# pashtari/factorizer

Measured on AMD Instinct MI355X. Metric: volumes/sec fwd+bwd, Swin Factorizer 128^3, higher is better.
Workload: dtype f32

## Files before the change

### factorizer_amd/_native.py

```python
from __future__ import annotations

import ctypes
import os
import threading

import torch

_HERE = os.path.dirname(os.path.abspath(__file__))
LIB_PATH = os.environ.get("FZ_LIB_PATH") or os.path.join(_HERE, "libfactorizer_hip.so")

FZ_OK = 0
FZ_E_UNSUPPORTED = -2
ABI_VERSION = 7
SOLVER_ID = {"mu": 0, "hals": 1, "cd": 2, "smu": 3}
STORE_F32, STORE_BF16 = 0, 1
PRODUCTS_DEFAULT, PRODUCTS_SPLIT_BF16, PRODUCTS_FP32_MFMA = 0, 1, 2
_products = threading.local()


def products() -> int:
    return getattr(_products, "value", PRODUCTS_DEFAULT)


class use_products:
# ... 171 lines not shown
    "fz_gcorr_supported": ([_i] * 5, _i),
    "fz_gcorr": ([_vp] * 5 + [_i] * 11 + [_f, _vp], _i),
    "fz_gcorr_wgrad_workspace_bytes": ([_i] * 10, _i64),
    "fz_gcorr_wgrad": ([_vp] * 4 + [_i] * 11 + [_vp], _i),
    "fz_gnmf_supported": ([_i, _i64, _i, _i, _i], _i),
    "fz_gnmf_workspace_bytes": ([_i64, _i, _i64, _i, _i, _i], _i64),
    "fz_gnmf_launches": ([_i, _i, _i], _i),
    "fz_gnmf_fwd": ([_vp] * 6 + [_i64, _i, _i64, _i, _i, _i, _f, _vp, _vp], _i),
    "fz_gnmf_bwd": ([_vp] * 7 + [_i64, _i, _i64, _i, _i, _i, _i, _f, _vp, _vp], _i),
    "fz_nmf_cf_supported": ([_i] * 11, _i),
    "fz_nmf_cf_fwd": ([_vp] * 4 + [_i] * 5 + [_c.POINTER(_i)] + [_i] * 5 + [_f, _i, _vp], _i),
    "fz_nmf_cf_bwd": ([_vp] * 5 + [_i] * 5 + [_c.POINTER(_i)] + [_i] * 7 + [_f, _i, _vp], _i),
    "fz_nmf_cf_factors_supported": ([_i] * 12 + [_c.POINTER(_i)], _i),
    "fz_nmf_cf_fwd_store_factors": ([_vp] * 5 + [_i] * 5 + [_c.POINTER(_i)] + [_i] * 3 + [_f, _i, _vp], _i),
    "fz_nmf_cf_fwd_from_factors": ([_vp] * 6 + [_i] * 5 + [_c.POINTER(_i)] * 2 + [_i] * 4 + [_f, _i, _vp], _i),
    "fz_nmf_pcf_supported": ([_i] * 11, _i),
    "fz_nmf_pcf_fwd": ([_vp] * 4 + [_i] * 8 + [_c.POINTER(_i)] + [_i] * 5 + [_f, _i, _vp], _i),
    "fz_nmf_pcf_bwd": ([_vp] * 5 + [_i] * 8 + [_c.POINTER(_i)] + [_i] * 7 + [_f, _i, _vp], _i),
    "fz_nmf_pcf_bwd_prefers_separate": ([_i] * 4, _i),
    "fz_act_add": ([_vp, _vp, _i64, _i, _vp], _i),
    "fz_mlp_pre_supported": ([_i, _i, _i64, _i], _i),
    "fz_mlp_drop_supported": ([_i, _i, _i64, _i], _i),
    "fz_mlp_chain_drop": ([_c.POINTER(MlpDesc), _c.POINTER(MlpDropout), _vp], _i),
    "fz_conv3_prologue_supported": ([_i] * 4, _i),
    "fz_conv3_fwd2": ([_vp] * 4 + [_i] * 8 + [_c.POINTER(BlockPrologue), _vp], _i),
    "fz_upcat2": ([_vp, _vp, _vp, _i, _vp, _vp, _vp] + [_i] * 7 + [_c.POINTER(BlockPrologue), _vp], _i),
    "fz_gemm": ([_c.POINTER(GemmDesc), _vp], _i),
    "fz_gemm_bx_enable": ([_i], _i),
    "fz_gemm_lnbwd_partials": ([_c.POINTER(GemmDesc)], _i64),
    "fz_reduce_rows": ([_vp, _i64, _i, _vp, _vp, _vp], _i),
# ... 65 lines not shown
```

### factorizer_amd/csrc/nmf_cf.h

```cpp
#pragma once
#include <cstdlib>

#include "fz_common.h"
#include "nmf_core.h"
#include "nmf_gram.h"

namespace fz {

struct CfGeom {
  int B, C, D, H, W;
  int h;
  int G0, G1, G2;
  int s0, s1, s2;
  int accumulate;
  int divisor;
  float gscale_div;
  int64_t plane;
  int ps0, ps1, ps2;
};

enum { CF_PLAIN = 0, CF_STORE_FACTORS = 1, CF_FROM_FACTORS = 2 };

struct CfWave {
  using F = float;
  int lane;
  __device__ __forceinline__ int col(int j) const {
    const int jp = j >> 2, e = j & 3;
    return (((jp * 4 + (lane >> 4)) * 8 + ((lane >> 1) & 7)) * 8) + (lane & 1) * 4 + e;
  }
  __device__ __forceinline__ float sum(float v) const { return wave_sum(v); }
  __device__ __forceinline__ void sum8(float (&v)[8]) const { wave_sum8(v, lane); }
  __device__ __forceinline__ void st_priv(float* base, int idx, float v) const { base[idx * 64 + lane] = v; }
  __device__ __forceinline__ float ld_priv(const float* base, int idx) const { return base[idx * 64 + lane]; }
  __device__ __forceinline__ void st_uni(float* base, int idx, float v) const {
    if (lane == 0) base[idx] = v;
  }
// ... 260 lines not shown
#pragma unroll
    for (int c = 0; c < 2; ++c) {
      const float4 a0 = *reinterpret_cast<const float4*>(S + c * 64 * TL::LW + own0);
      const float4 a1 = *reinterpret_cast<const float4*>(S + c * 64 * TL::LW + own1);
      x[2 * s + c][0] = a0.x; x[2 * s + c][1] = a0.y; x[2 * s + c][2] = a0.z; x[2 * s + c][3] = a0.w;
      x[2 * s + c][4] = a1.x; x[2 * s + c][5] = a1.y; x[2 * s + c][6] = a1.z; x[2 * s + c][7] = a1.w;
    }
    __syncthreads();
  }
}


template <typename AT>
int cf_bwd_gram_launch(const AT* t, const float* v0, const AT* ga, AT* gt, const CfGeom& q, int64_t nmat, int T, int G,
                       float eps, int xcd_remap, hipStream_t st);

}
```

### factorizer_amd/csrc/nmf_cf.hip

```cpp
#include "nmf_cf.h"

namespace fz {

template <int R, int SOLVER, int WPB, bool HALF, typename AT, int FORM>
__device__ __forceinline__ void cf_fwd_tile_body(const AT* __restrict__ t, const float* __restrict__ u0,
                                                 const float* __restrict__ v0, AT* __restrict__ out, float* vfac, float* ufac,
                                                 const CfGeom& q, const CfTileId& id, int T, float eps, float* S) {
  static_assert(FORM == CF_PLAIN || (R == 1 && WPB == 8 && !HALF), "the factor forms: rank 1, 8 patches per workgroup, W-axis shifts = 0 (mod 4)");
  using TL = CfTile<WPB>;
  const int tid = threadIdx.x, lane = tid & 63, wave = tid >> 6;
  int64_t base, V;
  unsigned off[2], off2[2];
  int lidx[2];
  cf_tile_decode<WPB>(q, id, tid, base, V, off, lidx, off2);
  const int own0 = cf_owner_lidx<WPB>(lane, wave, 0), own1 = cf_owner_lidx<WPB>(lane, wave, 1);

  float x[8][8];
#pragma unroll
  for (int dd = 0; dd < 8; ++dd)
#pragma unroll
    for (int k = 0; k < 2; ++k) {
      const float4 v = cf_ld4<HALF>(t + base + dd * V, off[k], off2[k]);
      x[dd][k * 4 + 0] = v.x; x[dd][k * 4 + 1] = v.y; x[dd][k * 4 + 2] = v.z; x[dd][k * 4 + 3] = v.w;
    }
// ... 397 lines not shown
  const int64_t nmat = (int64_t)B * q.h * q.G0 * q.G1 * q.G2;
  if (nmat >= (int64_t)1 << 31) return fail(FZ_E_UNSUPPORTED, "fz_nmf_cf: more than 2^31 matrices");
  const int per_wave = (R == 1 ? Hist<8, 8, 1>::floats(G) : Hist<8, 8, 2>::floats(G)) * (int)sizeof(float);
  if (per_wave > 160 * 1024) return fail(FZ_E_UNSUPPORTED, "fz_nmf_cf_bwd: history exceeds LDS");
  int wpb = 65536 / per_wave;
  if (wpb > 4) wpb = 4;
  if (wpb > 8) wpb = 8;
  if (wpb < 1) wpb = 1;
  const int xr = 1 | (tile_order() << 1);
  hipStream_t st = (hipStream_t)stream;
  const int tile = FZ_KNOB("FZ_CF_TILE_BWD").set ? FZ_KNOB("FZ_CF_TILE_BWD").val : 1;
  const bool half = (q.s2 % 4) != 0;
  if (half || (tile && (q.G2 % 4) == 0)) {
    const int twpb = (q.G2 % 4) == 0 ? 4 : 1;
    const bool gram_on = !(FZ_KNOB("FZ_CF_GRAM").set && FZ_KNOB("FZ_CF_GRAM").val == 0);
    const bool gram_wins = !(sizeof(AT) == 4 && accumulate && nmat >= 32768);
    if (gram_on && gram_wins && R == 1 && solver == FZ_SOLVER_HALS && relu_gate && G >= 1) {
      rc = cf_bwd_gram_launch<AT>(t, v0, ga, gt, q, nmat, T, G, eps, xr, st);
      if (rc != FZ_E_UNSUPPORTED) return rc;
    }
    const int tlds = (twpb == 4 ? CfTile<4>::STAGE_FLOATS : CfTile<1>::STAGE_FLOATS) * (int)sizeof(float) + per_wave * twpb;
    if (tlds > 160 * 1024) {
      if (half) return fail(FZ_E_UNSUPPORTED, "fz_nmf_cf_bwd: history exceeds LDS for a W-axis shift of 2 (mod 4)");
    } else {
      const unsigned nblk = (unsigned)(nmat / twpb);
#define FZ_CF_BWD_TILE(RR, SS, WW, HH)                                                                      \
  do {                                                                                                      \
    auto kern = nmf_cf_bwd_tile_kernel<RR, SS, WW, HH, AT>;                                                    \
    if (tlds > 65536)                                                                                       \
      FZ_HIP_OK(hipFuncSetAttribute(reinterpret_cast<const void*>(kern),                                    \
                                    hipFuncAttributeMaxDynamicSharedMemorySize, tlds));                     \
// ... 14 lines not shown
  dim3 grid((unsigned)((nmat + wpb - 1) / wpb)), block(64 * wpb);
#define FZ_CF_BWD(RR, SS)                                                                                 \
  do {                                                                                                    \
    auto kern = nmf_cf_bwd_kernel<RR, SS, AT>;                                                          \
    if (lds > 65536)                                                                                      \
      FZ_HIP_OK(hipFuncSetAttribute(reinterpret_cast<const void*>(kern),                                  \
                                    hipFuncAttributeMaxDynamicSharedMemorySize, lds));                    \
    hipLaunchKernelGGL(kern, grid, block, lds, st, t, u0, v0, ga, gt, q, nmat, T, G, eps, relu_gate, xr);     \
  } while (0)
  if (R == 1) { FZ_SOLVER_CASES(FZ_CF_BWD, 1); }
  else { FZ_SOLVER_CASES(FZ_CF_BWD, 2); }
  FZ_LAUNCH_CHECK();
  return FZ_OK;
}

extern "C" int fz_nmf_cf_bwd(const void* t, const float* u0, const float* v0, const void* ga, void* gt, int B,
                             int C, int D, int H, int W, const int* shift, int accumulate, int nshift,
                             int relu_gate, int R, int T, int Tgrad, int solver, float eps, int act_dtype,
                             fz_stream_t stream) {
  if (act_dtype == FZ_STORE_F32)
    return cf_bwd_launch<float>((const float*)t, u0, v0, (const float*)ga, (float*)gt, B, C, D, H, W, shift, accumulate,
                                nshift, relu_gate, R, T, Tgrad, solver, eps, stream);
  if (act_dtype == FZ_STORE_BF16)
    return cf_bwd_launch<bf16>((const bf16*)t, u0, v0, (const bf16*)ga, (bf16*)gt, B, C, D, H, W, shift, accumulate,
                               nshift, relu_gate, R, T, Tgrad, solver, eps, stream);
  return fail(FZ_E_ARG, "fz_nmf_cf_bwd: bad act_dtype");
}
```

### factorizer_amd/csrc/nmf_cf_gram.hip

```cpp
#include "nmf_cf.h"
#include "nmf_gram.h"

#ifndef FZ_GRAM_WAVES
#define FZ_GRAM_WAVES 3
#endif

namespace fz {

enum { CFG_HALVES = 0, CFG_RAW = 2 };

#ifdef FZ_PROBE_GRAM_NOMATH
#define FZ_GRAM_OUT_ROW(m, grow) probe_acc += grow[(m) & 7]
#else
#define FZ_GRAM_OUT_ROW(m, grow) P.out_row(m, grow)
#endif

template <typename AT> struct CfRaw;
template <> struct CfRaw<float> { using T = float4; };
template <> struct CfRaw<bf16> { using T = uint2; };

template <bool HALF>
__device__ __forceinline__ float4 cf_ld_raw(const float* p, unsigned o, unsigned o2) { return cf_ld4<HALF>(p, o, o2); }
template <bool HALF>
__device__ __forceinline__ uint2 cf_ld_raw(const bf16* p, unsigned o, unsigned o2) {
  if (HALF) {
    const unsigned a = *reinterpret_cast<const unsigned*>(cf_at(p, o)), b = *reinterpret_cast<const unsigned*>(cf_at(p, o2));
    return make_uint2(a, b);
  }
  return *reinterpret_cast<const uint2*>(cf_at(p, o));
}
__device__ __forceinline__ float4 cf_raw_f4(const float4& v) { return v; }
__device__ __forceinline__ float4 cf_raw_f4(const uint2& v) {
  return make_float4(__uint_as_float(v.x << 16), __uint_as_float(v.x & 0xffff0000u), __uint_as_float(v.y << 16),
                     __uint_as_float(v.y & 0xffff0000u));
}

template <int WPB, bool HALF, typename AT, int MODE>
__global__ __launch_bounds__(WPB * 64, WPB == 4 ? FZ_GRAM_WAVES : 1) void nmf_cf_bwd_gram_kernel(
    const AT* __restrict__ t, const float* __restrict__ v0, const AT* __restrict__ ga, AT* __restrict__ gt, CfGeom q,
    int T, int G, float eps, int xcd_remap) {
  extern __shared__ __attribute__((aligned(16))) float fz_lds_cfg[];
  using TL = CfTile<WPB>;
  using Raw = typename CfRaw<AT>::T;
  constexpr int NB = MODE == CFG_RAW ? 8 : 4;
  constexpr int IMG = 64 * TL::LW;
  float* S = fz_lds_cfg;
  const CfTileId id = cf_tile_id<WPB>(q, cf_logical_block(xcd_remap));
  const int tid = threadIdx.x, lane = tid & 63, wave = tid >> 6;
  int64_t base, V;
  unsigned off[2], off2[2];
  int lidx[2];
  cf_tile_decode<WPB>(q, id, tid, base, V, off, lidx, off2);
  const int own0 = cf_owner_lidx<WPB>(lane, wave, 0), own1 = cf_owner_lidx<WPB>(lane, wave, 1);
  float* hist = S + TL::STAGE_FLOATS + wave * gram_hist_floats(G - 1);

  float x[8][8];
#pragma unroll
  for (int dd = 0; dd < 8; ++dd)
#pragma unroll
    for (int k = 0; k < 2; ++k) {
      const float4 v = cf_ld4<HALF>(t + base + dd * V, off[k], off2[k]);
      x[dd][k * 4 + 0] = v.x; x[dd][k * 4 + 1] = v.y; x[dd][k * 4 + 2] = v.z; x[dd][k * 4 + 3] = v.w;
    }
  cf_to_owner<WPB>(S, lidx, own0, own1, x);

  CfWave w{lane};
  GramBwd<8, CfWave> P;
  Raw gq[NB][2];
  auto request_g = [&]() {
#pragma unroll
    for (int dd = 0; dd < NB; ++dd)
#pragma unroll
      for (int k = 0; k < 2; ++k) gq[dd][k] = cf_ld_raw<HALF>(ga + base + dd * V, off[k], off2[k]);
  };
#ifdef FZ_PROBE_GRAM_NOMATH
  float probe_acc = 0.f;
  request_g();
#else
  P.forward(w, x, v0, 8, 512, T, G, eps, hist, request_g);
#endif
  asm volatile("" : "+s"(base));
#pragma unroll
  for (int bt = 0; bt < 8 / NB; ++bt) {
#pragma unroll
    for (int s = 0; s < NB / 2; ++s) {
#pragma unroll
      for (int c = 0; c < 2; ++c)
#pragma unroll
        for (int k = 0; k < 2; ++k) *reinterpret_cast<float4*>(S + c * IMG + lidx[k]) = cf_raw_f4(gq[2 * s + c][k]);
      if (MODE == CFG_HALVES && bt == 0 && s == NB / 2 - 1) {
#pragma unroll
        for (int dd = 0; dd < NB; ++dd)
#pragma unroll
          for (int k = 0; k < 2; ++k) gq[dd][k] = cf_ld_raw<HALF>(ga + base + (NB + dd) * V, off[k], off2[k]);
      }
      __syncthreads();
#pragma unroll
      for (int c = 0; c < 2; ++c) {
        const float4 a0 = *reinterpret_cast<const float4*>(S + c * IMG + own0);
        const float4 a1 = *reinterpret_cast<const float4*>(S + c * IMG + own1);
        const float grow[8] = {a0.x, a0.y, a0.z, a0.w, a1.x, a1.y, a1.z, a1.w};
        FZ_GRAM_OUT_ROW(NB * bt + 2 * s + c, grow);
      }
      __syncthreads();
    }
  }
#ifdef FZ_PROBE_GRAM_NOMATH
#else
  P.reverse(w, x, 1.0f / q.gscale_div, [] {});
#endif
#pragma unroll
  for (int bt = 0; bt < 8 / NB; ++bt) {
#pragma unroll
    for (int s = 0; s < NB / 2; ++s) {
      Raw old[2][2];
      if (q.accumulate) {
#pragma unroll
        for (int c = 0; c < 2; ++c)
#pragma unroll
          for (int k = 0; k < 2; ++k) old[c][k] = cf_ld_raw<HALF>(gt + base + (NB * bt + 2 * s + c) * V, off[k], off2[k]);
      }
#pragma unroll
      for (int c = 0; c < 2; ++c) {
        const int m = NB * bt + 2 * s + c;
        float o[8];
#ifdef FZ_PROBE_GRAM_NOMATH
#pragma unroll
        for (int e = 0; e < 8; ++e) o[e] = x[m][e] + probe_acc;
#else
        float srow[8], gsm, ga1m;
        P.row_coeffs(w, m, srow, gsm, ga1m);
        P.gx_row(m, x, srow, gsm, ga1m, o);
#endif
#pragma unroll
        for (int e = 0; e < 8; ++e) o[e] = x[m][e] > 0.f ? o[e] : 0.f;
        *reinterpret_cast<float4*>(S + c * IMG + own0) = make_float4(o[0], o[1], o[2], o[3]);
        *reinterpret_cast<float4*>(S + c * IMG + own1) = make_float4(o[4], o[5], o[6], o[7]);
      }
      __syncthreads();
#pragma unroll
      for (int c = 0; c < 2; ++c)
#pragma unroll
        for (int k = 0; k < 2; ++k) {
          float4 z = *reinterpret_cast<const float4*>(S + c * IMG + lidx[k]);
          if (q.accumulate) {
            const float4 o = cf_raw_f4(old[c][k]);
            z.x += o.x; z.y += o.y; z.z += o.z; z.w += o.w;
          }
          cf_st4<HALF>(gt + base + (NB * bt + 2 * s + c) * V, off[k], off2[k], z);
        }
      __syncthreads();
    }
  }
}

template <typename AT>
int cf_bwd_gram_launch(const AT* t, const float* v0, const AT* ga, AT* gt, const CfGeom& q, int64_t nmat, int T, int G,
                       float eps, int xcd_remap, hipStream_t st) {
  const bool half = (q.s2 % 4) != 0;
#ifdef FZ_PROBE_GRAM_WPB
  const int twpb = (q.G2 % FZ_PROBE_GRAM_WPB) == 0 ? FZ_PROBE_GRAM_WPB : ((q.G2 % 4) == 0 ? 4 : 1);
#else
  const int twpb = (q.G2 % 4) == 0 ? 4 : 1;
#endif
  constexpr bool kF32 = sizeof(AT) == 4;
#ifdef FZ_PROBE_GRAM_WPB
  const int stage = twpb == FZ_PROBE_GRAM_WPB ? CfTile<FZ_PROBE_GRAM_WPB>::STAGE_FLOATS : (twpb == 4 ? CfTile<4>::STAGE_FLOATS : CfTile<1>::STAGE_FLOATS);
#else
// ... 10 lines not shown
#ifdef FZ_PROBE_GRAM_WPB
  if (!half && twpb == FZ_PROBE_GRAM_WPB) {
    auto kern = nmf_cf_bwd_gram_kernel<FZ_PROBE_GRAM_WPB, false, AT, kRegMode>;
    if (glds > 64 * 1024) FZ_HIP_OK(hipFuncSetAttribute(reinterpret_cast<const void*>(kern), hipFuncAttributeMaxDynamicSharedMemorySize, glds));
    FZ_CF_BWD_GRAM(FZ_PROBE_GRAM_WPB, false, kRegMode);
    FZ_LAUNCH_CHECK();
    return FZ_OK;
  }
#endif
  if (half) { if (twpb == 4) FZ_CF_BWD_GRAM(4, true, kRegMode); else FZ_CF_BWD_GRAM(1, true, kRegMode); }
  else if (twpb == 4) FZ_CF_BWD_GRAM(4, false, kRegMode);
  else return FZ_E_UNSUPPORTED;
  FZ_LAUNCH_CHECK();
  return FZ_OK;
}
template int cf_bwd_gram_launch<float>(const float*, const float*, const float*, float*, const CfGeom&, int64_t, int, int, float, int, hipStream_t);
template int cf_bwd_gram_launch<bf16>(const bf16*, const float*, const bf16*, bf16*, const CfGeom&, int64_t, int, int, float, int, hipStream_t);

}
```

### factorizer_amd/csrc/nmf_gram.h

```cpp
#pragma once

#include "nmf_core.h"

namespace fz {

FZ_HD int gram_hist_floats(int steps) { return 64 + (steps > 0 ? steps : 0) * 12; }

template <int NPL, class W>
struct GramBwd {
  using F = typename W::F;
  F vs[NPL];
  F gc[NPL];
  F vT[NPL];
  F gv[NPL];
  F col[8];
  F Kd[8];
  F gKd[8];
  F sd;
  F ud;
  F gsd, ga1d;
  F uT[8];
  F r;
  F binv;
  float eps, neps2;
// ... 186 lines not shown
#pragma unroll
      for (int k = 0; k < 8; ++k) gKd[k] = gKd[k] + gp * uk[k] + uo * gpk[k];
      un = uo;
    }
    ga1d = gud * binv;
  }

  FZ_HD void row_coeffs(W& w, int m, F (&srow)[8], F& gsm, F& ga1m) const {
#pragma unroll
    for (int k = 0; k < 8; ++k) srow[k] = w.grp_take(gKd[k], m);
    gsm = w.grp_take(gsd, m);
    ga1m = w.grp_take(ga1d, m);
  }
  FZ_HD void gx_row(int m, const F (&x)[8][NPL], const F (&srow)[8], const F& gsm, const F& ga1m, F (&out)[NPL]) const {
#pragma unroll
    for (int j = 0; j < NPL; ++j) {
      F acc = uT[m] * gc[j] + gsm;
      acc = acc + ga1m * vs[j];
#pragma unroll
      for (int k = 0; k < 8; ++k) acc = acc + srow[k] * x[k][j];
      out[j] = acc;
    }
  }
};

}
```

### factorizer_amd/functional.py

```python
from __future__ import annotations

import math
import os

import torch

from . import _native as N


def _dev_guard(t: torch.Tensor):
    return torch.cuda.device(t.device)


class KernelTimer:

    def __init__(self, only=None):
        self.records = []
        self.only = None if only is None else set(only)

    def launch(self, name, nbytes, fn, cols=0, flops=0):
        if self.only is not None and name not in self.only:
            return fn()
        s = torch.cuda.Event(enable_timing=True)
        e = torch.cuda.Event(enable_timing=True)
# ... 320 lines not shown

def nmf_cf_supported(geo: Geometry, R, T, G) -> bool:
    if len(geo.spatial) != 3 or any(s[2] % 2 for s in geo.shifts):
        return False
    return bool(N.lib().fz_nmf_cf_supported(geo.C, *geo.spatial, geo.d, *geo.patch, int(R), int(T), int(G)))


def nmf_cf_factors_supported(geo: Geometry, R, T, G) -> bool:
    if len(geo.spatial) != 3:
        return False
    k = (int(R), int(T), int(G))
    ok = geo._factors_ok.get(k)
    if ok is None:
        ok = geo._factors_ok[k] = bool(N.lib().fz_nmf_cf_factors_supported(geo.C, *geo.spatial, geo.d, *geo.patch, *k,
                                                                          geo.nshift, geo._carr))
    return ok


def nmf_pcf_supported(geo: Geometry, R, T, G) -> bool:
    if os.environ.get("FZ_NMF_PCF", "1") == "0":
        return False
    return bool(N.lib().fz_nmf_pcf_supported(geo.C, *geo.s3, geo.d, *geo.p3, int(R), int(T), int(G)))


def nmf_core_supported(geo: Geometry, R, T, G) -> bool:
    return nmf_cf_supported(geo, R, T, G) or nmf_pcf_supported(geo, R, T, G)


class FactCoreFn(torch.autograd.Function):

# ... 50 lines not shown
        t, u0, v0 = ctx.saved_tensors
        geo, T, G, solver, eps, relu_gate = ctx.cfg
        if G <= 0:
            return (torch.zeros_like(t),) + (None,) * 8
        ga = ga.contiguous()
        if ga.dtype != t.dtype:
            ga = ga.to(t.dtype)
        gt = torch.empty_like(t)
        B = t.shape[0]
        R = u0.shape[1]
        es = t.element_size()
        nb = 3 * es * t.numel()
        ad = N.act_dtype(t)
        hot = nmf_cf_supported(geo, R, T, G)
        with _dev_guard(t):
            for w, s in enumerate(geo.shifts3):
                arr = (N._i * 3)(*s)
                N.set_tile_order(w & 1)
                if hot:
                    rc = _timed(f"nmf_cf_bwd_{geo.C}x" + "x".join(str(v) for v in geo.spatial), nb + (es * t.numel() if w else 0), cols=t.numel() // geo.C, fn=lambda: N.lib().fz_nmf_cf_bwd(
                        t.data_ptr(), u0.data_ptr(), v0.data_ptr(), ga.data_ptr(), gt.data_ptr(), B, geo.C,
                        *geo.spatial, arr, int(w > 0), geo.nshift, int(relu_gate), R, T, G, N.SOLVER_ID[solver], eps,
                        ad, N.stream_ptr(t)))
                elif w > 0 and N.lib().fz_nmf_pcf_bwd_prefers_separate(*geo.p3, ad):
                    tmp = torch.empty_like(gt)
                    rc = _timed(f"nmf_pcf_bwd_{geo.C}x" + "x".join(str(v) for v in geo.spatial), nb, cols=t.numel() // geo.C, fn=lambda: N.lib().fz_nmf_pcf_bwd(
                        t.data_ptr(), u0.data_ptr(), v0.data_ptr(), ga.data_ptr(), tmp.data_ptr(), B, geo.C,
                        *geo.s3, *geo.p3, arr, 0, geo.nshift, int(relu_gate), R, T, G, N.SOLVER_ID[solver], eps,
                        ad, N.stream_ptr(t)))
                    N.check(rc, "fz_nmf_pcf_bwd")
# ... 251 lines not shown
```

### include/factorizer_hip.h

```cpp
#ifndef FACTORIZER_HIP_H
#define FACTORIZER_HIP_H

#include <stdint.h>

#ifdef __cplusplus
extern "C" {
#endif

#define FZ_OK 0
#define FZ_E_SHAPE (-1)
#define FZ_E_UNSUPPORTED (-2)
#define FZ_E_HIP (-3)
#define FZ_E_ARG (-4)

#define FZ_STORE_F32 0
#define FZ_STORE_BF16 1

#define FZ_SOLVER_MU 0
#define FZ_SOLVER_HALS 1
#define FZ_SOLVER_CD 2
#define FZ_SOLVER_SMU 3

typedef void* fz_stream_t;

// ... 41 lines not shown
                  int H, int W, const int* shift, int accumulate, int divisor, int R, int T,
                  int solver, float eps, int act_dtype, fz_stream_t stream);
int fz_nmf_cf_bwd(const void* t, const float* u0, const float* v0, const void* ga, void* gt, int B,
                  int C, int D, int H, int W, const int* shift, int accumulate, int nshift,
                  int relu_gate, int R, int T, int Tgrad, int solver, float eps, int act_dtype,
                  fz_stream_t stream);

int fz_nmf_cf_factors_supported(int C, int D, int H, int W, int d, int pd, int ph, int pw, int R, int T, int Tgrad,
                                int nshift, const int* shifts);
int fz_nmf_cf_fwd_store_factors(const void* t, const float* u0, const float* v0, float* vfac, float* ufac, int B,
                                int C, int D, int H, int W, const int* shift, int R, int T, int solver, float eps,
                                int act_dtype, fz_stream_t stream);
int fz_nmf_cf_fwd_from_factors(const void* t, const float* u0, const float* v0, const float* vfac, const float* ufac,
                               void* out, int B, int C, int D, int H, int W, const int* shift, const int* prev_shift,
                               int divisor, int R, int T, int solver, float eps, int act_dtype, fz_stream_t stream);

int fz_nmf_pcf_supported(int C, int D, int H, int W, int d, int pd, int ph, int pw, int R, int T, int Tgrad);
int fz_nmf_pcf_fwd(const void* t, const float* u0, const float* v0, void* out, int B, int C, int D, int H, int W,
                   int pd, int ph, int pw, const int* shift, int accumulate, int divisor, int R, int T, int solver,
                   float eps, int act_dtype, fz_stream_t stream);
int fz_nmf_pcf_bwd(const void* t, const float* u0, const float* v0, const void* ga, void* gt, int B, int C, int D,
                   int H, int W, int pd, int ph, int pw, const int* shift, int accumulate, int nshift, int relu_gate,
                   int R, int T, int Tgrad, int solver, float eps, int act_dtype, fz_stream_t stream);
int fz_nmf_pcf_bwd_prefers_separate(int pd, int ph, int pw, int act_dtype);
int fz_act_add(void* dst, const void* src, int64_t n, int act_dtype, fz_stream_t stream);

#define FZ_LOAD_PLAIN 0
#define FZ_LOAD_S2D 1
#define FZ_LOAD_K3 2
#define FZ_EPI_PLAIN 0
// ... 292 lines not shown
```

Before: 130.3.

## Fuse two-window NMF backward via stored per-patch factors instead of accumulate passes

Adds a factor-form backward for the shifted-window NMF. The first window's gram backward stores compact per-patch coefficients (gc image plus an 88-float cofactor record). The second window's kernel reconstructs the first window's input gradient from those factors and adds it in registers. This removes the separate accumulate read-modify-write of gt and one full pass over it, at the cost of extra factor storage, LDS staging and more arithmetic in the second kernel. The gram kernel body is moved into a shared include so both forms reuse it.

Measured after the change: 132.9 (median of 6 runs). 2.1% higher.

```diff
diff --git a/factorizer_amd/_native.py b/factorizer_amd/_native.py
--- a/factorizer_amd/_native.py
+++ b/factorizer_amd/_native.py
@@ -209,6 +209,9 @@
     "fz_nmf_cf_factors_supported": ([_i] * 12 + [_c.POINTER(_i)], _i),
     "fz_nmf_cf_fwd_store_factors": ([_vp] * 5 + [_i] * 5 + [_c.POINTER(_i)] + [_i] * 3 + [_f, _i, _vp], _i),
     "fz_nmf_cf_fwd_from_factors": ([_vp] * 6 + [_i] * 5 + [_c.POINTER(_i)] * 2 + [_i] * 4 + [_f, _i, _vp], _i),
+    "fz_nmf_cf_bwd_factors_supported": ([_i] * 14 + [_c.POINTER(_i)], _i),
+    "fz_nmf_cf_bwd_store_factors": ([_vp] * 5 + [_i] * 5 + [_c.POINTER(_i)] + [_i] * 3 + [_f, _i, _vp], _i),
+    "fz_nmf_cf_bwd_from_factors": ([_vp] * 6 + [_i] * 5 + [_c.POINTER(_i)] * 2 + [_i] * 3 + [_f, _i, _vp], _i),
     "fz_nmf_pcf_supported": ([_i] * 11, _i),
     "fz_nmf_pcf_fwd": ([_vp] * 4 + [_i] * 8 + [_c.POINTER(_i)] + [_i] * 5 + [_f, _i, _vp], _i),
     "fz_nmf_pcf_bwd": ([_vp] * 5 + [_i] * 8 + [_c.POINTER(_i)] + [_i] * 7 + [_f, _i, _vp], _i),
diff --git a/factorizer_amd/csrc/nmf_cf.h b/factorizer_amd/csrc/nmf_cf.h
--- a/factorizer_amd/csrc/nmf_cf.h
+++ b/factorizer_amd/csrc/nmf_cf.h
@@ -20,6 +20,7 @@
 };
 
 enum { CF_PLAIN = 0, CF_STORE_FACTORS = 1, CF_FROM_FACTORS = 2 };
+constexpr int CFG_COFAC = 88;
 
 struct CfWave {
   using F = float;
@@ -310,5 +311,8 @@
 template <typename AT>
 int cf_bwd_gram_launch(const AT* t, const float* v0, const AT* ga, AT* gt, const CfGeom& q, int64_t nmat, int T, int G,
                        float eps, int xcd_remap, hipStream_t st);
-
-}
+template <typename AT>
+int cf_bwd_gram_factors_launch(const AT* t, const float* v0, const AT* ga, AT* gt, float* gcfac, float* cofac, const CfGeom& q,
+                               int64_t nmat, int form, int T, int G, float eps, int xcd_remap, hipStream_t st);
+
+}
diff --git a/factorizer_amd/csrc/nmf_cf.hip b/factorizer_amd/csrc/nmf_cf.hip
--- a/factorizer_amd/csrc/nmf_cf.hip
+++ b/factorizer_amd/csrc/nmf_cf.hip
@@ -435,7 +435,7 @@
   if (half || (tile && (q.G2 % 4) == 0)) {
     const int twpb = (q.G2 % 4) == 0 ? 4 : 1;
     const bool gram_on = !(FZ_KNOB("FZ_CF_GRAM").set && FZ_KNOB("FZ_CF_GRAM").val == 0);
-    const bool gram_wins = !(sizeof(AT) == 4 && accumulate && nmat >= 32768);
+    const bool gram_wins = !(sizeof(AT) == 4 && accumulate && nmat >= 32768) || (FZ_KNOB("FZ_CF_GRAM").set && FZ_KNOB("FZ_CF_GRAM").val == 2);
     if (gram_on && gram_wins && R == 1 && solver == FZ_SOLVER_HALS && relu_gate && G >= 1) {
       rc = cf_bwd_gram_launch<AT>(t, v0, ga, gt, q, nmat, T, G, eps, xr, st);
       if (rc != FZ_E_UNSUPPORTED) return rc;
@@ -480,6 +480,74 @@
   return FZ_OK;
 }
 
+extern "C" int fz_nmf_cf_bwd_factors_supported(int C, int D, int H, int W, int d, int pd, int ph, int pw, int R, int T, int Tgrad,
+                                               int solver, int relu_gate, int nshift, const int* shifts) {
+  if (FZ_KNOB("FZ_CF_BWD_FACTORS").set && FZ_KNOB("FZ_CF_BWD_FACTORS").val == 0) return 0;
+  if (!fz_nmf_cf_factors_supported(C, D, H, W, d, pd, ph, pw, R, T, Tgrad, nshift, shifts)) return 0;
+  if (solver != FZ_SOLVER_HALS || !relu_gate) return 0;
+  if (T < 1 || Tgrad < T) return 0;
+  if ((C / 8) * (int64_t)(D / 8) * (H / 8) * (W / 8) >= ((int64_t)1 << 31)) return 0;
+  const int lds = (CfTile<4>::STAGE_FLOATS + 4 * gram_hist_floats(T - 1) + 4 * 8 * CFG_COFAC) * (int)sizeof(float);
+  return lds <= 64 * 1024 ? 1 : 0;
+}
+
+template <typename AT>
+static int cf_bwd_factors_launch(const AT* t, const float* v0, const AT* ga, AT* gt, float* gcfac, float* cofac, int B, int C,
+                                 int D, int H, int W, const int* shift, const int* prev_shift, int form, int nshift, int T,
+                                 int Tgrad, float eps, fz_stream_t stream, const char* who) {
+  CfGeom q;
+  int rc = cf_geom(q, B, C, D, H, W, shift, form == CF_FROM_FACTORS, 1);
+  if (rc != FZ_OK) return rc;
+  if (!t || !v0 || !ga || !gcfac || !cofac || (form == CF_FROM_FACTORS && (!gt || !prev_shift))) return fail(FZ_E_ARG, who);
+  if (W % 64) return fail(FZ_E_UNSUPPORTED, "fz_nmf_cf_bwd factor forms: W must be a multiple of 64");
+  if (nshift != 2) return fail(FZ_E_UNSUPPORTED, "fz_nmf_cf_bwd factor forms: exactly two windows");
+  if (T < 1 || Tgrad < T) return fail(FZ_E_UNSUPPORTED, "fz_nmf_cf_bwd factor forms: every iteration graded (1 <= T <= Tgrad)");
+  if (q.s2 % 4) return fail(FZ_E_UNSUPPORTED, "fz_nmf_cf_bwd factor forms: W-axis shift must be a multiple of 4");
+  if (form == CF_FROM_FACTORS) {
+    int ps[3];
+    cf_norm_shift(prev_shift, D, H, W, ps);
+    if (ps[2] % 4) return fail(FZ_E_UNSUPPORTED, "fz_nmf_cf_bwd factor forms: W-axis shift must be a multiple of 4");
+    q.ps0 = ps[0]; q.ps1 = ps[1]; q.ps2 = ps[2];
+  }
+  if (B == 0) return FZ_OK;
+  q.gscale_div = (float)nshift;
+  const int64_t nmat = (int64_t)B * q.h * q.G0 * q.G1 * q.G2;
+  if (nmat >= (int64_t)1 << 31) return fail(FZ_E_UNSUPPORTED, "fz_nmf_cf: more than 2^31 matrices");
+  const int xr = 1 | (tile_order() << 1);
+  rc = cf_bwd_gram_factors_launch<AT>(t, v0, ga, gt, gcfac, cofac, q, nmat, form, T, T, eps, xr, (hipStream_t)stream);
+  if (rc == FZ_E_UNSUPPORTED) return fail(rc, "fz_nmf_cf_bwd factor forms: history exceeds the LDS budget");
+  return rc;
+}
+
+extern "C" int fz_nmf_cf_bwd_store_factors(const void* t, const float* v0, const void* ga, float* gcfac, float* cofac, int B,
+                                           int C, int D, int H, int W, const int* shift, int nshift, int T, int Tgrad,
+                                           float eps, int act_dtype, fz_stream_t stream) {
+  const char* who = "fz_nmf_cf_bwd_store_factors: null pointer (t, v0, ga, gcfac or cofac)";
+  if (act_dtype == FZ_STORE_F32)
+    return cf_bwd_factors_launch<float>((const float*)t, v0, (const float*)ga, nullptr, gcfac, cofac, B, C, D, H, W, shift,
+                                        nullptr, CF_STORE_FACTORS, nshift, T, Tgrad, eps, stream, who);
+  if (act_dtype == FZ_STORE_BF16)
+    return cf_bwd_factors_launch<bf16>((const bf16*)t, v0, (const bf16*)ga, nullptr, gcfac, cofac, B, C, D, H, W, shift,
+                                       nullptr, CF_STORE_FACTORS, nshift, T, Tgrad, eps, stream, who);
+  return fail(FZ_E_ARG, "fz_nmf_cf_bwd_store_factors: bad act_dtype");
+}
+
+extern "C" int fz_nmf_cf_bwd_from_factors(const void* t, const float* v0, const void* ga, const float* gcfac,
+                                          const float* cofac, void* gt, int B, int C, int D, int H, int W, const int* shift,
+                                          const int* prev_shift, int nshift, int T, int Tgrad, float eps, int act_dtype,
+                                          fz_stream_t stream) {
+  const char* who = "fz_nmf_cf_bwd_from_factors: null pointer (t, v0, ga, gcfac, cofac, gt or prev_shift)";
+  if (act_dtype == FZ_STORE_F32)
+    return cf_bwd_factors_launch<float>((const float*)t, v0, (const float*)ga, (float*)gt, const_cast<float*>(gcfac),
+                                        const_cast<float*>(cofac), B, C, D, H, W, shift, prev_shift, CF_FROM_FACTORS, nshift, T,
+                                        Tgrad, eps, stream, who);
+  if (act_dtype == FZ_STORE_BF16)
+    return cf_bwd_factors_launch<bf16>((const bf16*)t, v0, (const bf16*)ga, (bf16*)gt, const_cast<float*>(gcfac),
+                                       const_cast<float*>(cofac), B, C, D, H, W, shift, prev_shift, CF_FROM_FACTORS, nshift, T,
+                                       Tgrad, eps, stream, who);
+  return fail(FZ_E_ARG, "fz_nmf_cf_bwd_from_factors: bad act_dtype");
+}
+
 extern "C" int fz_nmf_cf_bwd(const void* t, const float* u0, const float* v0, const void* ga, void* gt, int B,
                              int C, int D, int H, int W, const int* shift, int accumulate, int nshift,
                              int relu_gate, int R, int T, int Tgrad, int solver, float eps, int act_dtype,
diff --git a/factorizer_amd/csrc/nmf_cf_gram.hip b/factorizer_amd/csrc/nmf_cf_gram.hip
--- a/factorizer_amd/csrc/nmf_cf_gram.hip
+++ b/factorizer_amd/csrc/nmf_cf_gram.hip
@@ -35,123 +35,35 @@
                      __uint_as_float(v.y & 0xffff0000u));
 }
 
+template <typename AT>
+__device__ __forceinline__ float cf_as_stored(float v) {
+  if constexpr (sizeof(AT) == 2) {
+    const f32v4 f = {v, v, v, v};
+    const f32v4 r = __builtin_convertvector(__builtin_convertvector(f, bf16v4), f32v4);
+    return r[0];
+  }
+  return v;
+}
+
 template <int WPB, bool HALF, typename AT, int MODE>
 __global__ __launch_bounds__(WPB * 64, WPB == 4 ? FZ_GRAM_WAVES : 1) void nmf_cf_bwd_gram_kernel(
     const AT* __restrict__ t, const float* __restrict__ v0, const AT* __restrict__ ga, AT* __restrict__ gt, CfGeom q,
     int T, int G, float eps, int xcd_remap) {
   extern __shared__ __attribute__((aligned(16))) float fz_lds_cfg[];
-  using TL = CfTile<WPB>;
-  using Raw = typename CfRaw<AT>::T;
-  constexpr int NB = MODE == CFG_RAW ? 8 : 4;
-  constexpr int IMG = 64 * TL::LW;
-  float* S = fz_lds_cfg;
-  const CfTileId id = cf_tile_id<WPB>(q, cf_logical_block(xcd_remap));
-  const int tid = threadIdx.x, lane = tid & 63, wave = tid >> 6;
-  int64_t base, V;
-  unsigned off[2], off2[2];
-  int lidx[2];
-  cf_tile_decode<WPB>(q, id, tid, base, V, off, lidx, off2);
-  const int own0 = cf_owner_lidx<WPB>(lane, wave, 0), own1 = cf_owner_lidx<WPB>(lane, wave, 1);
-  float* hist = S + TL::STAGE_FLOATS + wave * gram_hist_floats(G - 1);
+  constexpr int FORM = CF_PLAIN;
+  float* const gcfac = nullptr;
+  float* const cofac = nullptr;
+#include "nmf_cf_gram_body.inc"
+}
 
-  float x[8][8];
-#pragma unroll
-  for (int dd = 0; dd < 8; ++dd)
-#pragma unroll
-    for (int k = 0; k < 2; ++k) {
-      const float4 v = cf_ld4<HALF>(t + base + dd * V, off[k], off2[k]);
-      x[dd][k * 4 + 0] = v.x; x[dd][k * 4 + 1] = v.y; x[dd][k * 4 + 2] = v.z; x[dd][k * 4 + 3] = v.w;
-    }
-  cf_to_owner<WPB>(S, lidx, own0, own1, x);
-
-  CfWave w{lane};
-  GramBwd<8, CfWave> P;
-  Raw gq[NB][2];
-  auto request_g = [&]() {
-#pragma unroll
-    for (int dd = 0; dd < NB; ++dd)
-#pragma unroll
-      for (int k = 0; k < 2; ++k) gq[dd][k] = cf_ld_raw<HALF>(ga + base + dd * V, off[k], off2[k]);
-  };
-#ifdef FZ_PROBE_GRAM_NOMATH
-  float probe_acc = 0.f;
-  request_g();
-#else
-  P.forward(w, x, v0, 8, 512, T, G, eps, hist, request_g);
-#endif
-  asm volatile("" : "+s"(base));
-#pragma unroll
-  for (int bt = 0; bt < 8 / NB; ++bt) {
-#pragma unroll
-    for (int s = 0; s < NB / 2; ++s) {
-#pragma unroll
-      for (int c = 0; c < 2; ++c)
-#pragma unroll
-        for (int k = 0; k < 2; ++k) *reinterpret_cast<float4*>(S + c * IMG + lidx[k]) = cf_raw_f4(gq[2 * s + c][k]);
-      if (MODE == CFG_HALVES && bt == 0 && s == NB / 2 - 1) {
-#pragma unroll
-        for (int dd = 0; dd < NB; ++dd)
-#pragma unroll
-          for (int k = 0; k < 2; ++k) gq[dd][k] = cf_ld_raw<HALF>(ga + base + (NB + dd) * V, off[k], off2[k]);
-      }
-      __syncthreads();
-#pragma unroll
-      for (int c = 0; c < 2; ++c) {
-        const float4 a0 = *reinterpret_cast<const float4*>(S + c * IMG + own0);
-        const float4 a1 = *reinterpret_cast<const float4*>(S + c * IMG + own1);
-        const float grow[8] = {a0.x, a0.y, a0.z, a0.w, a1.x, a1.y, a1.z, a1.w};
-        FZ_GRAM_OUT_ROW(NB * bt + 2 * s + c, grow);
-      }
-      __syncthreads();
-    }
-  }
-#ifdef FZ_PROBE_GRAM_NOMATH
-#else
-  P.reverse(w, x, 1.0f / q.gscale_div, [] {});
-#endif
-#pragma unroll
-  for (int bt = 0; bt < 8 / NB; ++bt) {
-#pragma unroll
-    for (int s = 0; s < NB / 2; ++s) {
-      Raw old[2][2];
-      if (q.accumulate) {
-#pragma unroll
-        for (int c = 0; c < 2; ++c)
-#pragma unroll
-          for (int k = 0; k < 2; ++k) old[c][k] = cf_ld_raw<HALF>(gt + base + (NB * bt + 2 * s + c) * V, off[k], off2[k]);
-      }
-#pragma unroll
-      for (int c = 0; c < 2; ++c) {
-        const int m = NB * bt + 2 * s + c;
-        float o[8];
-#ifdef FZ_PROBE_GRAM_NOMATH
-#pragma unroll
-        for (int e = 0; e < 8; ++e) o[e] = x[m][e] + probe_acc;
-#else
-        float srow[8], gsm, ga1m;
-        P.row_coeffs(w, m, srow, gsm, ga1m);
-        P.gx_row(m, x, srow, gsm, ga1m, o);
-#endif
-#pragma unroll
-        for (int e = 0; e < 8; ++e) o[e] = x[m][e] > 0.f ? o[e] : 0.f;
-        *reinterpret_cast<float4*>(S + c * IMG + own0) = make_float4(o[0], o[1], o[2], o[3]);
-        *reinterpret_cast<float4*>(S + c * IMG + own1) = make_float4(o[4], o[5], o[6], o[7]);
-      }
-      __syncthreads();
-#pragma unroll
-      for (int c = 0; c < 2; ++c)
-#pragma unroll
-        for (int k = 0; k < 2; ++k) {
-          float4 z = *reinterpret_cast<const float4*>(S + c * IMG + lidx[k]);
-          if (q.accumulate) {
-            const float4 o = cf_raw_f4(old[c][k]);
-            z.x += o.x; z.y += o.y; z.z += o.z; z.w += o.w;
-          }
-          cf_st4<HALF>(gt + base + (NB * bt + 2 * s + c) * V, off[k], off2[k], z);
-        }
-      __syncthreads();
-    }
-  }
+template <typename AT, int MODE, int FORM>
+__global__ __launch_bounds__(256, FZ_GRAM_WAVES) void nmf_cf_bwd_gram_fac_kernel(
+    const AT* __restrict__ t, const float* __restrict__ v0, const AT* __restrict__ ga, AT* __restrict__ gt,
+    float* __restrict__ gcfac, float* __restrict__ cofac, CfGeom q, int T, int G, float eps, int xcd_remap) {
+  extern __shared__ __attribute__((aligned(16))) float fz_lds_cfg[];
+  constexpr int WPB = 4;
+  constexpr bool HALF = false;
+#include "nmf_cf_gram_body.inc"
 }
 
 template <typename AT>
@@ -192,6 +104,27 @@
   FZ_LAUNCH_CHECK();
   return FZ_OK;
 }
+template <typename AT>
+int cf_bwd_gram_factors_launch(const AT* t, const float* v0, const AT* ga, AT* gt, float* gcfac, float* cofac, const CfGeom& q,
+                               int64_t nmat, int form, int T, int G, float eps, int xcd_remap, hipStream_t st) {
+  if ((q.s2 % 4) || (q.ps2 % 4) || (q.G2 % 4) || G != T || G < 1) return FZ_E_UNSUPPORTED;
+  int glds = (CfTile<4>::STAGE_FLOATS + 4 * gram_hist_floats(G - 1)) * (int)sizeof(float);
+  if (form == CF_FROM_FACTORS) glds += 4 * 8 * CFG_COFAC * (int)sizeof(float);
+  if (glds > 64 * 1024) return FZ_E_UNSUPPORTED;
+  const unsigned nblk = (unsigned)(nmat / 4);
+  constexpr int kRegMode = sizeof(AT) == 4 ? CFG_HALVES : CFG_RAW;
+  if (form == CF_STORE_FACTORS)
+    hipLaunchKernelGGL((nmf_cf_bwd_gram_fac_kernel<AT, kRegMode, CF_STORE_FACTORS>), dim3(nblk), dim3(256), glds, st, t, v0, ga,
+                       gt, gcfac, cofac, q, T, G, eps, xcd_remap);
+  else
+    hipLaunchKernelGGL((nmf_cf_bwd_gram_fac_kernel<AT, kRegMode, CF_FROM_FACTORS>), dim3(nblk), dim3(256), glds, st, t, v0, ga,
+                       gt, gcfac, cofac, q, T, G, eps, xcd_remap);
+  FZ_LAUNCH_CHECK();
+  return FZ_OK;
+}
+template int cf_bwd_gram_factors_launch<float>(const float*, const float*, const float*, float*, float*, float*, const CfGeom&, int64_t, int, int, int, float, int, hipStream_t);
+template int cf_bwd_gram_factors_launch<bf16>(const bf16*, const float*, const bf16*, bf16*, float*, float*, const CfGeom&, int64_t, int, int, int, float, int, hipStream_t);
+
 template int cf_bwd_gram_launch<float>(const float*, const float*, const float*, float*, const CfGeom&, int64_t, int, int, float, int, hipStream_t);
 template int cf_bwd_gram_launch<bf16>(const bf16*, const float*, const bf16*, bf16*, const CfGeom&, int64_t, int, int, float, int, hipStream_t);
 
diff --git a/factorizer_amd/csrc/nmf_cf_gram_body.inc b/factorizer_amd/csrc/nmf_cf_gram_body.inc
--- /dev/null
+++ b/factorizer_amd/csrc/nmf_cf_gram_body.inc
@@ -0,0 +1,207 @@
+  static_assert(FORM == CF_PLAIN || (WPB == 4 && !HALF), "the factor forms: 4 patches per workgroup, W-axis shifts = 0 (mod 4)");
+  using TL = CfTile<WPB>;
+  using Raw = typename CfRaw<AT>::T;
+  constexpr int NB = MODE == CFG_RAW ? 8 : 4;
+  constexpr int IMG = 64 * TL::LW;
+  float* S = fz_lds_cfg;
+  const CfTileId id = cf_tile_id<WPB>(q, cf_logical_block(xcd_remap));
+  const int tid = threadIdx.x, lane = tid & 63, wave = tid >> 6;
+  int64_t base, V;
+  unsigned off[2], off2[2];
+  int lidx[2];
+  cf_tile_decode<WPB>(q, id, tid, base, V, off, lidx, off2);
+  const int own0 = cf_owner_lidx<WPB>(lane, wave, 0), own1 = cf_owner_lidx<WPB>(lane, wave, 1);
+  float* hist = S + TL::STAGE_FLOATS + wave * gram_hist_floats(G - 1);
+
+  float x[8][8];
+#pragma unroll
+  for (int dd = 0; dd < 8; ++dd)
+#pragma unroll
+    for (int k = 0; k < 2; ++k) {
+      const float4 v = cf_ld4<HALF>(t + base + dd * V, off[k], off2[k]);
+      x[dd][k * 4 + 0] = v.x; x[dd][k * 4 + 1] = v.y; x[dd][k * 4 + 2] = v.z; x[dd][k * 4 + 3] = v.w;
+    }
+  const int64_t bh = (int64_t)id.b * q.h + id.hh;
+  const int64_t vol = (int64_t)q.D * q.H * q.W;
+  const float* co[2];
+  unsigned vcol[2];
+  if constexpr (FORM == CF_FROM_FACTORS) {
+    float* stage = S + TL::STAGE_FLOATS + WPB * gram_hist_floats(G - 1) + wave * (8 * CFG_COFAC);
+    const int gp[3] = {id.g0, id.g1, id.gq * WPB + wave}, sh[3] = {q.s0, q.s1, q.s2}, ps[3] = {q.ps0, q.ps1, q.ps2};
+    const int dim[3] = {q.D, q.H, q.W}, ng[3] = {q.G0, q.G1, q.G2};
+    int o[3], pa[3][2];
+#pragma unroll
+    for (int a = 0; a < 3; ++a) {
+      o[a] = gp[a] * 8 - sh[a] + ps[a];
+      if (o[a] < 0) o[a] += dim[a];
+      if (o[a] >= dim[a]) o[a] -= dim[a];
+      pa[a][0] = o[a] >> 3;
+      pa[a][1] = pa[a][0] + 1 == ng[a] ? 0 : pa[a][0] + 1;
+    }
+    const float* cp = cofac + bh * q.G0 * q.G1 * q.G2 * CFG_COFAC;
+#pragma unroll
+    for (int r = 0; r < 3; ++r) {
+      const int i = lane + 64 * r, lp = i / (CFG_COFAC / 4), c4 = i % (CFG_COFAC / 4);
+      if (i < 8 * (CFG_COFAC / 4)) {
+        const int pidx = (pa[0][(lp >> 2) & 1] * q.G1 + pa[1][(lp >> 1) & 1]) * q.G2 + pa[2][lp & 1];
+        *reinterpret_cast<float4*>(stage + lp * CFG_COFAC + c4 * 4) = ld4(cp + (int64_t)pidx * CFG_COFAC + c4 * 4);
+      }
+    }
+    __builtin_amdgcn_fence(__ATOMIC_ACQ_REL, "wavefront");
+    const int p12 = (lane >> 1) & 7, p2 = (lane & 1) * 4;
+    int c1 = o[1] + p12; if (c1 >= q.H) c1 -= q.H;
+    int c2 = o[2] + p2; if (c2 >= q.W) c2 -= q.W;
+    const int b1 = (c1 >> 3) != pa[1][0], b2 = (c2 >> 3) != pa[2][0];
+#pragma unroll
+    for (int jp = 0; jp < 2; ++jp) {
+      int c0 = o[0] + jp * 4 + (lane >> 4); if (c0 >= q.D) c0 -= q.D;
+      const int b0 = (c0 >> 3) != pa[0][0];
+      co[jp] = stage + (b0 * 4 + b1 * 2 + b2) * CFG_COFAC;
+      vcol[jp] = (unsigned)((((c0 & 7) * 8 + (c1 & 7)) * 8) + (c2 & 7));
+    }
+  }
+  cf_to_owner<WPB>(S, lidx, own0, own1, x);
+
+  CfWave w{lane};
+  GramBwd<8, CfWave> P;
+  Raw gq[NB][2];
+  auto request_g = [&]() {
+#pragma unroll
+    for (int dd = 0; dd < NB; ++dd)
+#pragma unroll
+      for (int k = 0; k < 2; ++k) gq[dd][k] = cf_ld_raw<HALF>(ga + base + dd * V, off[k], off2[k]);
+  };
+#ifdef FZ_PROBE_GRAM_NOMATH
+  float probe_acc = 0.f;
+  request_g();
+#else
+  P.forward(w, x, v0, 8, 512, T, G, eps, hist, request_g);
+#endif
+  asm volatile("" : "+s"(base));
+#pragma unroll
+  for (int bt = 0; bt < 8 / NB; ++bt) {
+#pragma unroll
+    for (int s = 0; s < NB / 2; ++s) {
+#pragma unroll
+      for (int c = 0; c < 2; ++c)
+#pragma unroll
+        for (int k = 0; k < 2; ++k) *reinterpret_cast<float4*>(S + c * IMG + lidx[k]) = cf_raw_f4(gq[2 * s + c][k]);
+      if (MODE == CFG_HALVES && bt == 0 && s == NB / 2 - 1) {
+#pragma unroll
+        for (int dd = 0; dd < NB; ++dd)
+#pragma unroll
+          for (int k = 0; k < 2; ++k) gq[dd][k] = cf_ld_raw<HALF>(ga + base + (NB + dd) * V, off[k], off2[k]);
+      }
+      __syncthreads();
+#pragma unroll
+      for (int c = 0; c < 2; ++c) {
+        const float4 a0 = *reinterpret_cast<const float4*>(S + c * IMG + own0);
+        const float4 a1 = *reinterpret_cast<const float4*>(S + c * IMG + own1);
+        const float grow[8] = {a0.x, a0.y, a0.z, a0.w, a1.x, a1.y, a1.z, a1.w};
+        FZ_GRAM_OUT_ROW(NB * bt + 2 * s + c, grow);
+      }
+      __syncthreads();
+    }
+  }
+  float4 gcq[2];
+  auto request_gc0 = [&] {
+    if constexpr (FORM == CF_FROM_FACTORS) {
+#pragma unroll
+      for (int k = 0; k < 2; ++k) gcq[k] = ld4(cf_at(gcfac + bh * vol, off[k]));
+    }
+  };
+#ifdef FZ_PROBE_GRAM_NOMATH
+  request_gc0();
+#else
+  P.reverse(w, x, 1.0f / q.gscale_div, request_gc0);
+#endif
+  if constexpr (FORM == CF_STORE_FACTORS) {
+    *reinterpret_cast<float4*>(S + own0) = make_float4(P.gc[0], P.gc[1], P.gc[2], P.gc[3]);
+    *reinterpret_cast<float4*>(S + own1) = make_float4(P.gc[4], P.gc[5], P.gc[6], P.gc[7]);
+    __syncthreads();
+    float* gp = gcfac + bh * vol;
+#pragma unroll
+    for (int k = 0; k < 2; ++k) st4(cf_at(gp, off[k]), *reinterpret_cast<const float4*>(S + lidx[k]));
+    if ((lane & 7) == 0) {
+      const int g = lane >> 3;
+      float* cp = cofac + ((((bh * q.G0 + id.g0) * q.G1 + id.g1) * q.G2 + id.gq * WPB + wave) * CFG_COFAC);
+      cp[g] = P.ud;
+      cp[8 + g] = P.gsd;
+      cp[16 + g] = P.ga1d;
+      st4(cp + 24 + g * 8, make_float4(P.gKd[0], P.gKd[1], P.gKd[2], P.gKd[3]));
+      st4(cp + 24 + g * 8 + 4, make_float4(P.gKd[4], P.gKd[5], P.gKd[6], P.gKd[7]));
+    }
+    return;
+  }
+  float gc0[8], vs0[8];
+  if constexpr (FORM == CF_FROM_FACTORS) {
+#pragma unroll
+    for (int k = 0; k < 2; ++k) *reinterpret_cast<float4*>(S + lidx[k]) = gcq[k];
+#pragma unroll
+    for (int jp = 0; jp < 2; ++jp) {
+#pragma unroll
+      for (int e = 0; e < 4; ++e) vs0[jp * 4 + e] = v0[vcol[jp] + e];
+    }
+    __syncthreads();
+    const float4 a0 = *reinterpret_cast<const float4*>(S + own0), a1 = *reinterpret_cast<const float4*>(S + own1);
+    gc0[0] = a0.x; gc0[1] = a0.y; gc0[2] = a0.z; gc0[3] = a0.w; gc0[4] = a1.x; gc0[5] = a1.y; gc0[6] = a1.z; gc0[7] = a1.w;
+    __syncthreads();
+  }
+#pragma unroll
+  for (int bt = 0; bt < 8 / NB; ++bt) {
+#pragma unroll
+    for (int s = 0; s < NB / 2; ++s) {
+      Raw old[2][2];
+      if (FORM == CF_PLAIN && q.accumulate) {
+#pragma unroll
+        for (int c = 0; c < 2; ++c)
+#pragma unroll
+          for (int k = 0; k < 2; ++k) old[c][k] = cf_ld_raw<HALF>(gt + base + (NB * bt + 2 * s + c) * V, off[k], off2[k]);
+      }
+#pragma unroll
+      for (int c = 0; c < 2; ++c) {
+        const int m = NB * bt + 2 * s + c;
+        float o[8];
+#ifdef FZ_PROBE_GRAM_NOMATH
+#pragma unroll
+        for (int e = 0; e < 8; ++e) o[e] = x[m][e] + probe_acc;
+#else
+        float srow[8], gsm, ga1m;
+        P.row_coeffs(w, m, srow, gsm, ga1m);
+        P.gx_row(m, x, srow, gsm, ga1m, o);
+#endif
+#pragma unroll
+        for (int e = 0; e < 8; ++e) o[e] = x[m][e] > 0.f ? o[e] : 0.f;
+        if constexpr (FORM == CF_FROM_FACTORS) {
+#pragma unroll
+          for (int jp = 0; jp < 2; ++jp) {
+            const float4 sa = *reinterpret_cast<const float4*>(co[jp] + 24 + m * 8);
+            const float4 sb = *reinterpret_cast<const float4*>(co[jp] + 24 + m * 8 + 4);
+            const float prow[8] = {sa.x, sa.y, sa.z, sa.w, sb.x, sb.y, sb.z, sb.w};
+            const float pu = co[jp][m], pgs = co[jp][8 + m], pga1 = co[jp][16 + m];
+#pragma unroll
+            for (int e = 0; e < 4; ++e) {
+              const int j = jp * 4 + e;
+              const float g0 = gram_gx_elem<float, 8>(pu, gc0[j], pgs, pga1, vs0[j], prow, x, j);
+              o[j] += cf_as_stored<AT>(x[m][j] > 0.f ? g0 : 0.f);
+            }
+          }
+        }
+        *reinterpret_cast<float4*>(S + c * IMG + own0) = make_float4(o[0], o[1], o[2], o[3]);
+        *reinterpret_cast<float4*>(S + c * IMG + own1) = make_float4(o[4], o[5], o[6], o[7]);
+      }
+      __syncthreads();
+#pragma unroll
+      for (int c = 0; c < 2; ++c)
+#pragma unroll
+        for (int k = 0; k < 2; ++k) {
+          float4 z = *reinterpret_cast<const float4*>(S + c * IMG + lidx[k]);
+          if (FORM == CF_PLAIN && q.accumulate) {
+            const float4 o = cf_raw_f4(old[c][k]);
+            z.x += o.x; z.y += o.y; z.z += o.z; z.w += o.w;
+          }
+          cf_st4<HALF>(gt + base + (NB * bt + 2 * s + c) * V, off[k], off2[k], z);
+        }
+      __syncthreads();
+    }
+  }
diff --git a/factorizer_amd/csrc/nmf_gram.h b/factorizer_amd/csrc/nmf_gram.h
--- a/factorizer_amd/csrc/nmf_gram.h
+++ b/factorizer_amd/csrc/nmf_gram.h
@@ -5,6 +5,16 @@
 namespace fz {
 
 FZ_HD int gram_hist_floats(int steps) { return 64 + (steps > 0 ? steps : 0) * 12; }
+
+template <class F, int NPL>
+FZ_HD F gram_gx_elem(const F& uTm, const F& gcj, const F& gsm, const F& ga1m, const F& vsj, const F (&srow)[8],
+                     const F (&x)[8][NPL], int j) {
+  F acc = uTm * gcj + gsm;
+  acc = acc + ga1m * vsj;
+#pragma unroll
+  for (int k = 0; k < 8; ++k) acc = acc + srow[k] * x[k][j];
+  return acc;
+}
 
 template <int NPL, class W>
 struct GramBwd {
@@ -224,13 +234,7 @@
   }
   FZ_HD void gx_row(int m, const F (&x)[8][NPL], const F (&srow)[8], const F& gsm, const F& ga1m, F (&out)[NPL]) const {
 #pragma unroll
-    for (int j = 0; j < NPL; ++j) {
-      F acc = uT[m] * gc[j] + gsm;
-      acc = acc + ga1m * vs[j];
-#pragma unroll
-      for (int k = 0; k < 8; ++k) acc = acc + srow[k] * x[k][j];
-      out[j] = acc;
-    }
+    for (int j = 0; j < NPL; ++j) out[j] = gram_gx_elem<F, NPL>(uT[m], gc[j], gsm, ga1m, vs[j], srow, x, j);
   }
 };
 
diff --git a/factorizer_amd/functional.py b/factorizer_amd/functional.py
--- a/factorizer_amd/functional.py
+++ b/factorizer_amd/functional.py
@@ -358,6 +358,17 @@
     if ok is None:
         ok = geo._factors_ok[k] = bool(N.lib().fz_nmf_cf_factors_supported(geo.C, *geo.spatial, geo.d, *geo.patch, *k,
                                                                           geo.nshift, geo._carr))
+    return ok
+
+
+def nmf_cf_bwd_factors_supported(geo: Geometry, R, T, G, solver, relu_gate) -> bool:
+    if len(geo.spatial) != 3:
+        return False
+    k = ("bwd", int(R), int(T), int(G), solver, bool(relu_gate))
+    ok = geo._factors_ok.get(k)
+    if ok is None:
+        ok = geo._factors_ok[k] = bool(N.lib().fz_nmf_cf_bwd_factors_supported(
+            geo.C, *geo.spatial, geo.d, *geo.patch, *k[1:4], N.SOLVER_ID[solver], int(k[5]), geo.nshift, geo._carr))
     return ok
 
 
@@ -438,6 +449,25 @@
         ad = N.act_dtype(t)
         hot = nmf_cf_supported(geo, R, T, G)
         with _dev_guard(t):
+            if hot and nmf_cf_bwd_factors_supported(geo, R, T, G, solver, relu_gate):
+                gcfac = torch.empty((B, geo.h, *geo.spatial), device=t.device, dtype=torch.float32)
+                cofac = torch.empty((B * geo.h * geo.G, 88), device=t.device, dtype=torch.float32)
+                s0, s1 = ((N._i * 3)(*s) for s in geo.shifts3)
+                key = f"nmf_cf_bwd_{geo.C}x" + "x".join(str(v) for v in geo.spatial)
+                nf = 4 * (t.numel() // 8) + 4 * cofac.numel()
+                st = N.stream_ptr(t)
+                N.set_tile_order(0)
+                rc = _timed(key, 2 * es * t.numel() + nf, cols=t.numel() // geo.C, fn=lambda: N.lib().fz_nmf_cf_bwd_store_factors(
+                    t.data_ptr(), v0.data_ptr(), ga.data_ptr(), gcfac.data_ptr(), cofac.data_ptr(), B, geo.C, *geo.spatial, s0,
+                    geo.nshift, T, G, eps, ad, st))
+                N.check(rc, "fz_nmf_cf_bwd_store_factors")
+                N.set_tile_order(1)
+                rc = _timed(key, 3 * es * t.numel() + nf, cols=t.numel() // geo.C, fn=lambda: N.lib().fz_nmf_cf_bwd_from_factors(
+                    t.data_ptr(), v0.data_ptr(), ga.data_ptr(), gcfac.data_ptr(), cofac.data_ptr(), gt.data_ptr(), B, geo.C,
+                    *geo.spatial, s1, s0, geo.nshift, T, G, eps, ad, st))
+                N.check(rc, "fz_nmf_cf_bwd_from_factors")
+                N.set_tile_order(0)
+                return (gt,) + (None,) * 8
             for w, s in enumerate(geo.shifts3):
                 arr = (N._i * 3)(*s)
                 N.set_tile_order(w & 1)
diff --git a/include/factorizer_hip.h b/include/factorizer_hip.h
--- a/include/factorizer_hip.h
+++ b/include/factorizer_hip.h
@@ -79,6 +79,15 @@
 int fz_nmf_cf_fwd_from_factors(const void* t, const float* u0, const float* v0, const float* vfac, const float* ufac,
                                void* out, int B, int C, int D, int H, int W, const int* shift, const int* prev_shift,
                                int divisor, int R, int T, int solver, float eps, int act_dtype, fz_stream_t stream);
+
+int fz_nmf_cf_bwd_factors_supported(int C, int D, int H, int W, int d, int pd, int ph, int pw, int R, int T, int Tgrad,
+                                    int solver, int relu_gate, int nshift, const int* shifts);
+int fz_nmf_cf_bwd_store_factors(const void* t, const float* v0, const void* ga, float* gcfac, float* cofac, int B, int C,
+                                int D, int H, int W, const int* shift, int nshift, int T, int Tgrad, float eps,
+                                int act_dtype, fz_stream_t stream);
+int fz_nmf_cf_bwd_from_factors(const void* t, const float* v0, const void* ga, const float* gcfac, const float* cofac,
+                               void* gt, int B, int C, int D, int H, int W, const int* shift, const int* prev_shift,
+                               int nshift, int T, int Tgrad, float eps, int act_dtype, fz_stream_t stream);
 
 int fz_nmf_pcf_supported(int C, int D, int H, int W, int d, int pd, int ph, int pw, int R, int T, int Tgrad);
 int fz_nmf_pcf_fwd(const void* t, const float* u0, const float* v0, void* out, int B, int C, int D, int H, int W,
```
